# yli421/koopman-mpc-portfolio-rebalancing

Hardware: AMD Instinct MI355X
Metric: MPC window-solves/sec (batched backtest) at 1/2/4/8 MI355X vs host-CPU ref (higher is better)
Workload: dtype f32 rollout (fp32 GEMMs as three exact bf16 planes); mixed f32->f64 IPM solve (float32 phase to mu 3e-5, float64 finish: stopping rule, status and W in float64); 1 GPU; C3 (BASELINE configs[2]): 65536 windows/GPU, 100 assets, latent 256, H=10, obs 2000, GenericKM enc [1024,1024], L1-turnover MPC c=1e-3 tau=0.2 no-short; windows_per_gpu=65536, parallelism=1 GPU, no collective

## Files before the change

### koopman_mpc_portfolio_rebalancing_amd/csrc/kmpc_ipm_body.inc

```
    if constexpr (PH == 3) {
        if (reinterpret_cast<const int*>(args.warm + (size_t)b * args.warm_floats)[0] != 3) return;
    }
    const int nw = GL < 64 ? 1 : (MAXT <= 128 ? NWM : (int)(blockDim.x / WAVE));
    Reducer<HM, NWM, GL, Real> R(sh, nw);
    Thread<HM, MAXT, FL, CS, QL, GL, Real> T;
    T.bind_cold();
    T.H = EXACT ? HM : args.H;
    T.N = args.N;
    T.i = gvt<GL>();
    T.act = T.i < args.N;
    T.set_case(!args.allow_short, (args.c > Real(0.0)) || (args.tau > Real(0.0)), args.tau > Real(0.0));
    T.tau = args.tau;
    const int H = T.H, N = T.N;
    const double* wp = args.wp + (size_t)b * N;
    const float* yh = args.yhat + (size_t)yb * H * N;
    T.wpi = T.act ? wp[T.i] : Real(0.0);

    Real mx = Real(0.0);
    bool finite = true;
    bool r_zero = false;
    {
        Real rs[HM];
#pragma unroll
        for (int t = 0; t < HM; ++t) {
            T.m[t] = rs[t] = Real(0.0);
            if (T.act && t < H) {
                const float r = np_expf(yh[t * N + T.i]);
                T.m[t] = (Real)((double)r - 1.0);
                rs[t] = (Real)r;
                finite = finite && isfinite(T.m[t]);
            }
        }
        if (T.act) finite = finite && isfinite(T.wpi);
        R.periods(rs);
#pragma unroll
        for (int t = 0; t < HM; ++t) {
            r_zero = r_zero || (t < H && rs[t] == Real(0.0));
            if (T.act && t < H && rs[t] > Real(0.0) && rs[t] < Real(TINY_PERIOD))
                T.m[t] = (Real)((double)np_expf(yh[t * N + T.i]) / (double)rs[t] - 1.0);
            if (T.act && t < H) mx = fmax(mx, fabs(T.m[t]));
        }
        if (gvt<GL>() == 0) {
#pragma unroll
            for (int t = 0; t < HM; ++t)
                sh.lsc[t] = (t < H && rs[t] > Real(0.0) && rs[t] < Real(TINY_PERIOD)) ? (Real)log((double)rs[t]) : Real(0.0);
        }
    }
    mx = R.max1(mx);
    const Real nonfinite = R.max1(finite ? Real(0.0) : Real(1.0));
    Real sig = fmax(mx, Real(args.c));
    if (!(sig > Real(0.0))) sig = Real(1.0);
    T.sig = sig;
    T.isig = Real(1.0) / sig;
    T.irsig = Real(1.0) / sqrt(sig);
    T.c = Real(args.c) / sig;

    int status = KMPC_STATUS_SOLVER_ERROR;
    int it = 0;
    double* wout = args.wout + (size_t)b * (args.return_full ? H * N : N);
    const int tw = args.return_full ? H : 1;
    double best_obj = __builtin_nan("");
    bool handoff = false;
    int it0 = 0;

    if (nonfinite == Real(0.0) && isfinite(args.c) && isfinite(args.tau)) {
        if (r_zero) {
            status = KMPC_STATUS_INFEASIBLE;
        } else if (args.allow_short && !T.hs) {
            Real msum[HM];
#pragma unroll
            for (int t = 0; t < HM; ++t) msum[t] = (T.act && t < H) ? T.m[t] : Real(0.0);
            R.periods(msum);
            Real spread = Real(0.0);
#pragma unroll
            for (int t = 0; t < HM; ++t)
                if (T.act && t < H) spread = fmax(spread, fabs(T.m[t] - msum[t] / N));
            spread = R.max1(spread);
            if (spread == Real(0.0)) {
                const Real swp = R.sum1(T.act ? T.wpi : Real(0.0));
#pragma unroll
                for (int t = 0; t < HM; ++t) T.w[t] = swp != Real(0.0) ? T.wpi / swp : Real(1.0) / N;
                if constexpr (PH != 1) best_obj = record_best<HM, NWM>(T, R, wout, yh, args.c, tw);
                status = KMPC_STATUS_OPTIMAL;
            } else {
// ... 274 lines not shown
                }
                KMPC_PH(ph, 6);
            }
            __syncthreads();
            if (PH != 1 && best < huge_of<Real>()) {
                Real f = Real(0.0);
                for (int t = 0; t < H; ++t) f += log(sh.best_rw[t]) + sh.lsc[t] - args.c * sh.best_l1[t];
                best_obj = f;
            }
            if (best <= Real(1e-7)) status = KMPC_STATUS_OPTIMAL;
            else if (best <= Real(1e-4)) status = KMPC_STATUS_OPTIMAL_INACCURATE;
            else if (min_pr > Real(1e-6)) status = KMPC_STATUS_INFEASIBLE;
            else status = KMPC_STATUS_SOLVER_ERROR;
        }
    }
    if constexpr (PH == 1) {
        float* rec = args.warm + (size_t)b * args.warm_floats;
#ifdef KMPC_REG_HANDOFF
        hand_flag = handoff;
        if (handoff) {
#if KMPC_REG_HANDOFF_ON == 2
            float* hl = reinterpret_cast<float*>(kmpc_cold);
            const int ln = hand_lane<CS>();
#pragma unroll
            for (int t = 0; t < HM; ++t) {
                hl[(0 * HM + t) * CS + ln] = T.w[t];
                hl[(1 * HM + t) * CS + ln] = T.s[t];
                hl[(2 * HM + t) * CS + ln] = T.l1[t];
                hl[(3 * HM + t) * CS + ln] = T.l2[t];
                hl[(4 * HM + t) * CS + ln] = T.l3[t];
            }
            if (gvt<GL>() < HM) {
                hl[5 * HM * CS + gvt<GL>()] = sh.z4[gvt<GL>()];
                hl[5 * HM * CS + HM + gvt<GL>()] = sh.l4[gvt<GL>()];
                hl[5 * HM * CS + 2 * HM + gvt<GL>()] = sh.nu[gvt<GL>()];
            }
#else
#pragma unroll
            for (int t = 0; t < HM; ++t) {
                hand_w[t] = T.w[t];
                hand_s[t] = T.s[t];
                hand_l1[t] = T.l1[t];
                hand_l2[t] = T.l2[t];
                hand_l3[t] = T.l3[t];
            }
            if (gvt<GL>() < HM) {
                hand_z4 = sh.z4[gvt<GL>()];
                hand_l4 = sh.l4[gvt<GL>()];
                hand_nu = sh.nu[gvt<GL>()];
            }
#endif
        }
        if (false) {
#else
        if (handoff) {
#endif
            float* st = rec + WARM_HEAD;
#pragma unroll
            for (int t = 0; t < HM; ++t) {
                if (T.act && t < H) {
                    const int k = t * N + T.i;
                    st[k] = T.w[t];
                    st[H * N + k] = T.s[t];
                    st[2 * H * N + k] = T.l1[t];
                    st[3 * H * N + k] = T.l2[t];
                    st[4 * H * N + k] = T.l3[t];
                }
            }
            if (gvt<GL>() < H) {
                const int t = gvt<GL>();
                st[5 * H * N + t] = sh.z4[t];
                st[5 * H * N + H + t] = sh.l4[t];
                st[5 * H * N + 2 * H + t] = sh.nu[t];
            }
        }
        if (gvt<GL>() == 0) {
            int* hd = reinterpret_cast<int*>(rec);
            hd[0] = handoff ? 1 : 0;
            hd[1] = it;
        }
        return;
    }
    __syncthreads();
    const bool ok = status == KMPC_STATUS_OPTIMAL || status == KMPC_STATUS_OPTIMAL_INACCURATE;
    if (!ok && T.act) {
#pragma unroll
        for (int t = 0; t < HM; ++t)
            if (t < tw) wout[t * N + T.i] = T.wpi;
    }
    if (gvt<GL>() == 0) {
        args.obj[b] = ok ? best_obj : __builtin_nan("");
        args.status[b] = status;
        if constexpr (PH >= 2) {
            int* hd = reinterpret_cast<int*>(args.warm + (size_t)b * args.warm_floats);
            it0 = hd[1];
            if (PH == 2 && hd[0] == 1 && status != KMPC_STATUS_OPTIMAL) {
                hd[0] = 3;
                hd[1] = it + it0;
            }
        }
        if (args.iters) args.iters[b] = it + it0;
    }
```

### koopman_mpc_portfolio_rebalancing_amd/csrc/kmpc_solve_c3.hip

```cpp
#include "kmpc_solve_kernel.h"
#include "kmpc_bt_run.h"

#ifndef KMPC_REG_HANDOFF_ON
#define KMPC_REG_HANDOFF_ON 1
#endif

namespace kmpc {
template <int CS>
__device__ __forceinline__ int hand_lane() { const int t = (int)threadIdx.x; return t < CS ? t : CS - 1; }
}

namespace kmpc {
namespace {
template <int HM, int MAXT, bool EXACT, int FL, int CS, bool QL, int GL>
__global__ void __launch_bounds__(MAXT) __attribute__((amdgpu_waves_per_eu(1))) ipm_mixed_kernel(SolveArgs args) {
    constexpr int NWM = MAXT / WAVE;
    __shared__ union U {
        Shared<HM, NWM, float> f;
        Shared<HM, NWM, double> d;
    } shu;
    const int b = blockIdx.x;
    if (b >= args.B) return;
    const int yb = b;
#if KMPC_REG_HANDOFF_ON
    static_assert(KMPC_REG_HANDOFF_ON != 2 || (5 * HM * CS + 3 * HM) * 4 <= cold_bytes<HM, MAXT, CS, QL, GL, FL, double>(),
                  "the handoff fits the float64 cold arrays' LDS");
#if KMPC_REG_HANDOFF_ON == 1
    float hand_w[HM], hand_s[HM], hand_l1[HM], hand_l2[HM], hand_l3[HM];
    float hand_z4 = 1.0f, hand_l4 = 0.0f, hand_nu = 0.0f;
#endif
    bool hand_flag = false;
#define KMPC_REG_HANDOFF
#endif
    [&]() __attribute__((always_inline)) {
        constexpr int PH = 1;
        using Real = float;
        auto& sh = shu.f;
#include "kmpc_ipm_body.inc"
    }();
    __syncthreads();
    [&]() __attribute__((always_inline)) {
        constexpr int PH = 2;
        using Real = double;
        auto& sh = shu.d;
#include "kmpc_ipm_body.inc"
    }();
#undef KMPC_REG_HANDOFF
}
}

#ifndef KMPC_MIXED_FUSED
#define KMPC_MIXED_FUSED 1
#endif

size_t mixed_warm_floats(int H, int N) {
    return KMPC_MIXED_FUSED && KMPC_REG_HANDOFF_ON ? (size_t)WARM_HEAD : warm_stride(H, N);
}

int launch_ipm_c3(const SolveArgs& a, hipStream_t stream) {
    if (a.warm && KMPC_MIXED_FUSED) {
        const size_t lds = cold_bytes<10, 128, QL_CS, true, 64, 7, double>();
        hipLaunchKernelGGL((ipm_mixed_kernel<10, 128, true, 7, QL_CS, true, 64>), dim3(a.B), dim3(128), lds, stream, a);
        int rc = hipGetLastError() == hipSuccess ? KMPC_OK : KMPC_ERR_LAUNCH;
        if (rc == KMPC_OK) rc = launch_one<10, 128, true, 7, QL_CS, true, 64, 3>(a, 128, stream);
        return rc;
    }
    if (a.warm) {
        int rc = launch_one<10, 128, true, 7, QL_CS, true, 64, 1>(a, 128, stream);
        if (rc == KMPC_OK) rc = launch_one<10, 128, true, 7, QL_CS, true, 64, 2>(a, 128, stream);
        if (rc == KMPC_OK) rc = launch_one<10, 128, true, 7, QL_CS, true, 64, 3>(a, 128, stream);
        return rc;
    }
    return launch_one<10, 128, true, 7, QL_CS, true>(a, 128, stream);
}

int launch_bt_run_c3(const SolveArgs& a, int n_steps, int n_real, const float* yhat, const float* realized,
                     int step0, int S, double c, double* weights, double* value, double* hist, hipStream_t stream) {
    return launch_bt_run_one<10, 128, true, 7, QL_CS, true>(a, n_steps, n_real, yhat, realized, step0, S, c, weights,
                                                           value, hist, stream);
}
}

#ifdef KMPC_STATS
extern "C" int kmpc_debug_stats_c3(unsigned long long* out, int reset) { return kmpc::debug_stats_tu(out, reset); }
#endif
```

### koopman_mpc_portfolio_rebalancing_amd/csrc/kmpc_solve_c3sw.hip

```cpp
#include "kmpc_solve_kernel.h"
#include "kmpc_bt_sweep.h"

namespace kmpc {
int launch_bt_sweep_c3(const SolveArgs& a, const SweepLaunch& l, hipStream_t stream) {
    return launch_bt_sweep_one<10, 128, true, 7, QL_CS, true>(a, l, stream);
}
}
```

### koopman_mpc_portfolio_rebalancing_amd/csrc/kmpc_solve_kernel.h

```cpp
#pragma once
#include <hip/hip_runtime.h>
#include <math.h>
#include <stdint.h>

#include <type_traits>
#include <utility>

#include "kmpc_internal.h"
#include "kmpc_npexp.h"
#include "kmpc_solve_args.h"

namespace kmpc {

constexpr int WAVE = 64;
#ifdef KMPC_STATS
__device__ unsigned long long g_stats[2];
__device__ unsigned long long g_phase[16];
#ifndef KMPC_STATS_REAL
#define KMPC_STATS_REAL 0
#endif
struct PhaseClock {
    unsigned long long last;
    bool on;
    __device__ __forceinline__ void start(int real_bytes) {
// ... 235 lines not shown
}
__device__ __forceinline__ float bcast(float v, int src) { return as_f(__builtin_amdgcn_readlane(as_i(v), src)); }

template <int GL>
__device__ __forceinline__ int gvt() { return GL == 64 ? (int)threadIdx.x : (int)(threadIdx.x & (GL - 1)); }
template <int GL>
__device__ __forceinline__ int grp() { return GL == 64 ? 0 : (int)(threadIdx.x / GL); }
template <int GL>
__device__ __forceinline__ int glane() { return (int)(threadIdx.x & ((GL == 64 ? WAVE : GL) - 1)); }
template <int GL>
__device__ __forceinline__ int gwave() { return GL == 64 ? (int)(threadIdx.x / WAVE) : 0; }

template <int GL, class T>
__device__ __forceinline__ T group_sum(T v) {
    if constexpr (GL > 32) v = pair_sum<32>(v);
    if constexpr (GL > 16) v = pair_sum<16>(v);
    v = pair_sum<8>(v); v = pair_sum<4>(v); v = pair_sum<2>(v); v = pair_sum<1>(v);
    return v;
}
template <int GL, class T>
__device__ __forceinline__ T group_max(T v) {
    if constexpr (GL > 32) v = fmax(v, partner<32>(v));
    if constexpr (GL > 16) v = fmax(v, partner<16>(v));
    v = fmax(v, partner<8>(v)); v = fmax(v, partner<4>(v)); v = fmax(v, partner<2>(v)); v = fmax(v, partner<1>(v));
    return v;
}
template <int GL, class T>
__device__ __forceinline__ T group_min(T v) {
    if constexpr (GL > 32) v = fmin(v, partner<32>(v));
    if constexpr (GL > 16) v = fmin(v, partner<16>(v));
    v = fmin(v, partner<8>(v)); v = fmin(v, partner<4>(v)); v = fmin(v, partner<2>(v)); v = fmin(v, partner<1>(v));
    return v;
}
template <int C>
__device__ __forceinline__ double dpp_f64(double v) {
    const int2 x = as_i2(v);
    return as_f64(__builtin_amdgcn_mov_dpp(x.x, C, 0xf, 0xf, false),
                  __builtin_amdgcn_mov_dpp(x.y, C, 0xf, 0xf, false));
}
__device__ __forceinline__ double row_bcast(double v, int j) {
    switch (j & 15) {
        case 0: return dpp_f64<0x150>(v);
        case 1: return dpp_f64<0x151>(v);
        case 2: return dpp_f64<0x152>(v);
        case 3: return dpp_f64<0x153>(v);
        case 4: return dpp_f64<0x154>(v);
        case 5: return dpp_f64<0x155>(v);
        case 6: return dpp_f64<0x156>(v);
        case 7: return dpp_f64<0x157>(v);
        case 8: return dpp_f64<0x158>(v);
        case 9: return dpp_f64<0x159>(v);
        case 10: return dpp_f64<0x15a>(v);
        case 11: return dpp_f64<0x15b>(v);
        case 12: return dpp_f64<0x15c>(v);
        case 13: return dpp_f64<0x15d>(v);
        case 14: return dpp_f64<0x15e>(v);
        default: return dpp_f64<0x15f>(v);
    }
}
template <int C>
__device__ __forceinline__ float dpp_f32(float v) {
    return as_f(__builtin_amdgcn_mov_dpp(as_i(v), C, 0xf, 0xf, false));
}
__device__ __forceinline__ float row_bcast(float v, int j) {
    switch (j & 15) {
        case 0: return dpp_f32<0x150>(v);
        case 1: return dpp_f32<0x151>(v);
        case 2: return dpp_f32<0x152>(v);
        case 3: return dpp_f32<0x153>(v);
        case 4: return dpp_f32<0x154>(v);
        case 5: return dpp_f32<0x155>(v);
        case 6: return dpp_f32<0x156>(v);
        case 7: return dpp_f32<0x157>(v);
        case 8: return dpp_f32<0x158>(v);
        case 9: return dpp_f32<0x159>(v);
        case 10: return dpp_f32<0x15a>(v);
        case 11: return dpp_f32<0x15b>(v);
        case 12: return dpp_f32<0x15c>(v);
        case 13: return dpp_f32<0x15d>(v);
        case 14: return dpp_f32<0x15e>(v);
        default: return dpp_f32<0x15f>(v);
    }
}
template <int GL, class T>
__device__ __forceinline__ T gbcast(T v, int src) {
    if constexpr (GL == 64) {
        return bcast(v, src);
    } else if constexpr (GL == 16) {
        return row_bcast(v, src);
    } else {
        static_assert(GL == 32, "lane group of 16, 32 or 64");
        T a = row_bcast(v, src), b = a;
        swap16(a, b);
        return (src & 16) ? b : a;
    }
}

#ifndef KMPC_OPAQUE_LANE
#define KMPC_OPAQUE_LANE 1
#endif
#ifndef KMPC_RS_BANK
#define KMPC_RS_BANK 1
#endif
template <int M, int D, class T>
__device__ __forceinline__ void rs_level(T (&v)[M], int& n, int& slot) {
    if (n > 1) {
        const int h = n >> 1;
        const bool up = (threadIdx.x & D) != 0;
#pragma unroll
        for (int j = 0; j < (M > 1 ? M / 2 : 1); ++j) {
            if (j < h) {
                if constexpr (D == 32 || D == 16) {
                    T a = v[j], b = v[j + h];
                    if constexpr (D == 32) swap32(a, b); else swap16(a, b);
                    v[j] = a + b;
                } else if constexpr (KMPC_RS_BANK && (D == 8 || D == 4) && sizeof(T) == 4) {
                    constexpr int ctrl = D == 8 ? 0x140 : 0x141;
                    constexpr int lowm = D == 8 ? 0x3 : 0x5, upm = D == 8 ? 0xc : 0xa;
                    const int lo = as_i(v[j]), hi = as_i(v[j + h]);
                    const T t = as_f(__builtin_amdgcn_update_dpp(hi, lo, ctrl, 0xf, lowm, false));
                    const T u = as_f(__builtin_amdgcn_update_dpp(lo, hi, ctrl, 0xf, upm, false));
                    v[j] = t + u;
                } else if constexpr (KMPC_RS_BANK && (D == 8 || D == 4)) {
                    constexpr int ctrl = D == 8 ? 0x140 : 0x141;
                    constexpr int lowm = D == 8 ? 0x3 : 0x5, upm = D == 8 ? 0xc : 0xa;
                    const int2 lo = as_i2(v[j]), hi = as_i2(v[j + h]);
                    const double t = as_f64(__builtin_amdgcn_update_dpp(hi.x, lo.x, ctrl, 0xf, lowm, false),
                                            __builtin_amdgcn_update_dpp(hi.y, lo.y, ctrl, 0xf, lowm, false));
                    const double u = as_f64(__builtin_amdgcn_update_dpp(lo.x, hi.x, ctrl, 0xf, upm, false),
                                            __builtin_amdgcn_update_dpp(lo.y, hi.y, ctrl, 0xf, upm, false));
                    v[j] = t + u;
                } else {
                    const T lo = v[j], hi = v[j + h];
                    const T send = up ? lo : hi;
                    const T keep = up ? hi : lo;
                    v[j] = keep + dpp_partner<D>(send);
                }
            }
        }
        slot += up ? h : 0;
        n = h;
    } else {
        v[0] = pair_sum<D>(v[0]);
    }
}

template <int M, int GL = 64, class T>
__device__ __forceinline__ int wave_reduce_scatter(T (&v)[M]) {
    static_assert(M <= GL, "one slot per lane at most");
    int slot = 0, n = M;
    if constexpr (GL > 32) rs_level<M, 32>(v, n, slot);
    if constexpr (GL > 16) rs_level<M, 16>(v, n, slot);
    rs_level<M, 8>(v, n, slot);
    rs_level<M, 4>(v, n, slot);
    rs_level<M, 2>(v, n, slot);
    rs_level<M, 1>(v, n, slot);
    return slot;
}

template <class Real, int HM, int CS, bool LDS, int GL = 64>
struct Cold;
template <class Real, int HM, int CS, int GL>
struct Cold<Real, HM, CS, false, GL> {
    Real v[HM];
    __device__ __forceinline__ void bind(int) {}
    __device__ __forceinline__ Real operator[](int t) const { return v[t]; }
    __device__ __forceinline__ void set(int t, Real x) { v[t] = x; }
};
extern __shared__ double kmpc_cold[];
template <class Real, int HM, int CS, int GL>
struct Cold<Real, HM, CS, true, GL> {
    static constexpr int GS = GL < 64 ? CS / (64 / GL) : CS;
    int k;
    __device__ __forceinline__ void bind(int kk) { k = kk; }
    __device__ __forceinline__ static int lane() {
        const int tid = (int)threadIdx.x;
        if constexpr (GL < 64) {
            const int g = tid / GL, i = tid % GL;
            return g * GS + (i < GS ? i : GS - 1);
        } else {
            return tid < CS ? tid : CS - 1;
        }
// ... 640 lines not shown
            } else {
                r0[t] = r1[t] = Real(0.0);
            }
            rn = fmax(rn, fmax(fabs(r0[t]), fabs(r1[t])));
            if (gvt<TH::GLN>() == 0 && t < H) rn = fmax(rn, fabs(sh.b6[t] - sdw[t]));
            nl2 = (t < H) ? dl2 : Real(0.0);
            nl3 = (t < H) ? dl3 : Real(0.0);
        }
        if (!T.act) rn = Real(0.0);
        rn = R.max1(rn);
        KMPC_PH(np, 14);
        if (rn <= Real(REFINE_RTOL) * bn) break;
        if (gvt<TH::GLN>() < HM) {
            const int t = gvt<TH::GLN>();
            sh.lb5[t] = Real(0.0);
            sh.lb6[t] = (t < H) ? sh.b6[t] - sdw[t] : Real(0.0);
        }
        __syncthreads();
    }
#ifdef KMPC_STATS
    if (threadIdx.x == 0 && (KMPC_STATS_REAL == 0 || sizeof(Real) == KMPC_STATS_REAL)) {
        atomicAdd(&g_stats[0], (unsigned long long)r);
        atomicAdd(&g_stats[1], 1ull);
    }
#endif
    if (gvt<TH::GLN>() < HM) {
        const int t = gvt<TH::GLN>();
        const Real st = T.hs ? pxa * sh.isp1[t] : Real(0.0);
        const bool on = T.ht && t < H;
        sh.dz4[t] = on ? -st + sh.rg4[t] : Real(0.0);
        sh.dl4[t] = on ? (sh.b5[t] + sh.l4[t] * st) * sh.iz4[t] : Real(0.0);
    }
    KMPC_PH(np, 15);
}

template <int HM, int NWM, class TH, class Real = typename TH::real_t>
__device__ __forceinline__ Real max_step(const TH& T, Shared<HM, NWM, typename TH::real_t>& sh, Reducer<HM, NWM, TH::GLN, typename TH::real_t>& R,
                                           Real& c1, Real& c2) {
    const int H = T.H;
    Real a = huge_of<Real>(), mdw[HM];
    c1 = c2 = Real(0.0);
    Real DL1[HM], DL2[HM], DL3[HM];
    T.dual_dirs_all(DL1, DL2, DL3);
    Real qx = Real(0.0);
#pragma unroll
    for (int t = 0; t < HM; ++t) {
        mdw[t] = Real(0.0);
        if (t < H) {
            const Real dl1 = DL1[t], dl2 = DL2[t], dl3 = DL3[t];
            const Real d = T.w[t] - T.wprev(t);
            const Real dd = T.dw[t] - (t ? T.dw[t - 1] : Real(0.0));
            if (T.hw) {
                qx = fmax(qx, -T.dw[t] * T.iw[t]);
                a = to_bound(T.l1[t], dl1, a);
                c1 += T.w[t] * dl1 + T.l1[t] * T.dw[t];
                c2 += T.dw[t] * dl1;
            }
            if (T.hs) {
                const Real x2 = T.s[t] - d, dx2 = T.ds[t] - dd, x3 = T.s[t] + d, dx3 = T.ds[t] + dd;
                qx = fmax(qx, fmax(-dx2 * T.iz2[t], -dx3 * T.iz3[t]));
                a = to_bound(T.l2[t], dl2, a);
                a = to_bound(T.l3[t], dl3, a);
                c1 += x2 * dl2 + T.l2[t] * dx2 + x3 * dl3 + T.l3[t] * dx3;
                c2 += dx2 * dl2 + dx3 * dl3;
            }
            mdw[t] = T.m[t] * T.dw[t];
        }
    }
    if (qx > Real(0.0)) a = fmin(a, rcp_nr(qx));
    if (T.ht && (int)gvt<TH::GLN>() < H) {
        const int t = gvt<TH::GLN>();
        a = to_bound(sh.z4[t], sh.dz4[t], a);
        a = to_bound(sh.l4[t], sh.dl4[t], a);
        c1 += sh.z4[t] * sh.dl4[t] + sh.l4[t] * sh.dz4[t];
        c2 += sh.dz4[t] * sh.dl4[t];
    }
    a = R.periods_min_sums(mdw, a, c1, c2);
    Real qr = Real(0.0);
#pragma unroll
    for (int t = 0; t < HM; ++t)
        if (t < H) qr = fmax(qr, -mdw[t] * sh.iden[t]);
    if (qr > Real(0.0)) a = fmin(a, rcp_nr(qr));
    return a;
}

template <int HM, int NWM, class TH, class Real = typename TH::real_t>
__device__ __forceinline__ bool factor(TH& T, Shared<HM, NWM, typename TH::real_t>& sh, Reducer<HM, NWM, TH::GLN, typename TH::real_t>& R,
                                      PhaseClock& ph) {
    constexpr int KM = 3 * HM;
    constexpr int MC = Shared<HM, NWM>::MC;
    constexpr int RW = Shared<HM, NWM>::RW;
    const int H = T.H;
    Real E[HM], W1[HM], sp[HM];
#pragma unroll
    for (int t = 0; t < HM; ++t) {
        W1[t] = E[t] = T.P[t] = sp[t] = Real(0.0);
        Real iw = Real(0.0), iz2 = Real(0.0), iz3 = Real(0.0);
        if (T.act && t < H) {
            const Real d = T.w[t] - T.wprev(t);
            if (T.hw) { iw = rcp_nr(T.w[t]); W1[t] = T.l1[t] * iw; }
            if (T.hs) {
                iz2 = rcp_nr(T.s[t] - d);
                iz3 = rcp_nr(T.s[t] + d);
                const Real al = T.l2[t] * iz2, be = T.l3[t] * iz3;
                const Real P = rcp_nr(al + be);
                T.P[t] = P;
                E[t] = Real(4.0) * al * be * P;
                sp[t] = P;
            }
        }
        T.iw.set(t, iw);
        T.iz2.set(t, iz2);
        T.iz3.set(t, iz3);
    }
    const Real st_own = R.own1(sp);
    if (gvt<TH::GLN>() < HM) {
        const int t = gvt<TH::GLN>();
        const Real st = st_own;
        const Real ga = (T.ht && t < H) ? sh.l4[t] / sh.z4[t] : Real(0.0);
        const Real i1 = Real(1.0) / (Real(1.0) + ga * st);
        sh.rho[t] = (T.ht && t < H) ? ga * i1 : Real(0.0);
        sh.sr[t] = sqrt(sh.rho[t]);
        sh.sp[t] = t < H ? st : Real(0.0);
        sh.isp1[t] = i1;
        if (t == 0) sh.flag = 0;
    }
    bool ok = true;
    Real iDd[HM], Lr[HM];
    {
        Real pi = W1[0] + E[0];
#pragma unroll
        for (int t = 0; t < HM; ++t) {
            iDd[t] = Real(1.0);
            Lr[t] = Real(0.0);
            if (T.act && t < H) {
                if (t > 0) {
                    Lr[t] = E[t] * iDd[t - 1];
                    pi = W1[t] + Lr[t] * pi;
                }
                const Real dd = pi + ((t + 1 < HM && t + 1 < H) ? E[t + 1] : Real(0.0));
                ok = ok && (dd > Real(0.0)) && (dd < huge_of<Real>());
                iDd[t] = rcp_nr(dd);
            }
        }
#pragma unroll
        for (int t = 0; t < HM; ++t) {
            T.iDd.set(t, iDd[t]);
            T.Lr.set(t, Lr[t]);
        }
    }
    Real dq[HM];
#pragma unroll
    for (int k = HM - 1; k >= 0; --k) {
        Real v = Real(0.0);
        if (T.act && k < H) {
            v = iDd[k];
            if (k + 1 < HM) v += Lr[k + 1] * Lr[k + 1] * dq[k + 1];
        }
        dq[k] = v;
    }
    __syncthreads();
    if (!ok) sh.flag = 1;
    auto al = [&](int t) -> Real { return t < H ? T.m[t] * sh.iden[t] * T.irsig : Real(0.0); };
    auto ep = [&](int t) -> Real { return (t < H && T.ht) ? sh.sr[t] * T.bma(t) * T.P[t] : Real(0.0); };
    const int lane = glane<TH::GLN>(), wv = gwave<TH::GLN>();
    KMPC_PH(ph, 1);
// ... 63 lines not shown
        }
        __syncthreads();
#pragma unroll
        for (int k = 0; k < SPT; ++k) {
            const int s = gvt<TH::GLN>() + k * (TH::GLN == 64 ? (int)blockDim.x : TH::GLN);
            if (s < NS) {
                const int jl = kGramTab<HM>.v[s];
                const int j = jl & 255, l = jl >> 8;
                sh.G[j * KM + l] = tot[k];
                sh.G[l * KM + j] = tot[k];
            }
        }
    } else {
        Real qp[HM];
    #pragma unroll
        for (int r = 0; r < HM; ++r) qp[r] = Real(0.0);
        KMPC_PH(ph, 1);
        for (int c = 0; c < H; ++c) {
            Real qc[HM];
            Real dqc = Real(0.0), ac = Real(0.0), ec = Real(0.0);
    #pragma unroll
            for (int k = 0; k < HM; ++k) if (k == c) { dqc = dq[k]; ac = al(k); ec = ep(k); }
            {
                Real nxt = Real(0.0);
    #pragma unroll
                for (int r = HM - 1; r >= 0; --r) {
                    const Real v = (r == c) ? dqc : ((r < c && r + 1 < HM) ? Lr[r + 1] * nxt : Real(0.0));
                    qc[r] = v;
                    nxt = v;
                }
            }
            Real qcm1 = Real(0.0);
    #pragma unroll
            for (int k = 0; k + 1 < HM; ++k) if (k + 1 == c) qcm1 = qc[k];
            Real* rb = &sh.red[R.buf][0][0];
    #pragma unroll
            for (int k = 0; k < 3; ++k) {
                const Real cl = (k == 0) ? ac : ((k == 1) ? ec : Real(1.0));
                Real v[MC];
    #pragma unroll
                for (int q = 0; q < MC; ++q) {
                    Real x = Real(0.0);
                    if (q < KM) {
                        const int ty = q / HM, tj = q % HM;
                        if (tj <= c) {
                            Real base = qc[tj];
                            if (ty == 1 && tj >= 1) base -= qc[tj - 1];
                            if (k == 1) {
                                Real cross = (tj < c) ? qp[tj] : qcm1;
                                if (ty == 1 && tj >= 1) cross -= qp[tj - 1];
                                if (c == 0) cross = Real(0.0);
                                base -= cross;
                            }
                            const Real cj = (ty == 0) ? al(tj) : ((ty == 1) ? ep(tj) : Real(1.0));
                            x = cj * (cl * base);
                        }
                    }
                    v[q] = x;
                }
                const int slot = wave_reduce_scatter<MC, TH::GLN>(v);
                if ((lane & ((TH::GLN / MC) - 1)) == 0) rb[wv * RW + k * MC + slot] = v[0];
            }
            __syncthreads();
            for (int q = gvt<TH::GLN>(); q < 3 * MC; q += (TH::GLN == 64 ? (int)blockDim.x : TH::GLN)) {
                const int tyl = q / MC, j = q % MC;
                if (j < KM) {
                    const int tyj = j / HM, tj = j % HM;
                    if (tj < c || (tj == c && tyj <= tyl)) {
                        Real s = Real(0.0);
                        for (int w = 0; w < R.nw; ++w) s += rb[w * RW + q];
                        const int l = tyl * HM + c;
                        sh.G[j * KM + l] = s;
                        sh.G[l * KM + j] = s;
                    }
                }
            }
            R.buf ^= Shared<HM, NWM>::NB - 1;
    #pragma unroll
            for (int r = 0; r < HM; ++r) qp[r] = qc[r];
        }
    }
    __syncthreads();
    KMPC_PH(ph, 2);
    Real* col = &sh.red[0][0][0];
    if (gvt<TH::GLN>() < WAVE) {
        int r = lane;
#if KMPC_OPAQUE_LANE
        asm volatile("" : "+v"(r));
#endif
        const bool rused = r < KM && (r % HM) < H && (r / HM != 1 || T.ht);
        Real g[KM];
#pragma unroll
        for (int k = 0; k < KM; ++k) {
            const bool kused = (k % HM) < H && (k / HM != 1 || T.ht);
            Real v = (r < KM && k <= r && rused && kused) ? sh.G[r * KM + k] : Real(0.0);
            if (k == r) v += (k / HM < 2 || !rused) ? Real(1.0) : Real(0.0);
            g[k] = v;
        }
        bool bad = false;
        Real dinv = Real(0.0);
#pragma unroll
        for (int j = 0; j < KM; ++j) {
            const Real u = g[j];
            Real cv[KM];
            if (j + 1 < KM) {
                col[r] = u;
                __builtin_amdgcn_wave_barrier();
#pragma unroll
                for (int k = j + 1; k < KM; ++k) cv[k] = col[k];
            }
            const Real d = gbcast<TH::GLN>(u, j);
            bad = bad || !(d > Real(0.0)) || !(d < huge_of<Real>());
            const Real dm = fmax(d, tiny_of<Real>());
            Real id;
            if constexpr (sizeof(Real) == 8) {
                id = __builtin_amdgcn_rcp(dm);
                id = fma(id, fma(-dm, id, Real(1.0)), id);
                id = fma(id, fma(-dm, id, Real(1.0)), id);
            } else {
                id = __builtin_amdgcn_rcpf(dm);
            }
            const Real l = (r > j) ? u * id : Real(0.0);
            if (r == j) dinv = id;
            g[j] = l;
            if (j + 1 < KM) {
                __builtin_amdgcn_sched_barrier(0);
#pragma unroll
                for (int k = j + 1; k < KM; ++k) g[k] = fma(-l, cv[k], g[k]);
                __builtin_amdgcn_wave_barrier();
            }
        }
        if (r < KM) {
#pragma unroll
            for (int k = 0; k < KM; ++k) {
                const Real v = k < r ? g[k] : Real(0.0);
                sh.G[r * KM + k] = v;
            }
            sh.gid[r] = dinv;
        }
        if (bad && lane == 0) sh.flag = 1;
    }
    __syncthreads();
    KMPC_PH(ph, 3);
    return sh.flag == 0;
}

template <int HM, int NWM, class TH, class Real = typename TH::real_t>
__device__ __forceinline__ Real record_best(const TH& T, Reducer<HM, NWM, TH::GLN, typename TH::real_t>& R, double* wout,
                                              const float* yh, Real c, int tw) {
    const int H = T.H, N = T.N;
    Real rw[HM], l1n[HM];
#pragma unroll
    for (int t = 0; t < HM; ++t) {
        rw[t] = l1n[t] = Real(0.0);
        if (T.act && t < H) {
            if (t < tw) wout[t * N + T.i] = T.w[t];
            rw[t] = (Real(1.0) + T.m[t]) * T.w[t];
            l1n[t] = fabs(T.w[t] - T.wprev(t));
        }
    }
    R.periods(rw, l1n);
    Real f = Real(0.0);
#pragma unroll
    for (int t = 0; t < HM; ++t)
        if (t < H) f += log(rw[t]) + R.sh.lsc[t] - c * l1n[t];
    return f;
}

template <int HM, int MAXT, bool EXACT, int FL = -1, int CS = MAXT, bool QL = false, int GL = 64, int PH = 0>
__global__ void __launch_bounds__(MAXT)
__attribute__((amdgpu_waves_per_eu(PH == 1 ? KMPC_F32_WPE : (HM <= KMPC_WPE2_HM ? 2 : 1)))) ipm_kernel(SolveArgs args) {
    static_assert(3 * HM <= GL, "Schur system must fit one lane group");
    static_assert(GL == 64 || MAXT == 64, "lane groups pack one-wave blocks");
    using Real = std::conditional_t<PH == 1, float, double>;
    constexpr int NWM = MAXT / WAVE;
    constexpr int WPB = GL == 64 ? 1 : 64 / GL;
    static_assert(!cold_in_lds<HM, MAXT, CS, QL, GL, FL, Real>() ||
                  sizeof(Shared<HM, NWM, Real>) * WPB <= 9 * HM * HM * 8 + 16 * 1024, "cold_in_lds() LDS estimate");
    static_assert(sizeof(Shared<HM, NWM, Real>) * WPB + cold_bytes<HM, MAXT, CS, QL, GL, FL, Real>() <= 160 * 1024,
                  "LDS of one workgroup");
    __shared__ Shared<HM, NWM, Real> shv[WPB];
    auto& sh = shv[grp<GL>()];
    const int b = blockIdx.x * WPB + grp<GL>();
    if (b >= args.B) return;
    const int yb = b;
// ... 76 lines not shown
```

Baseline: 842,900 windows/s.

## Fuse float64 retry phase into mixed kernel and use DPP broadcasts in LDL

The float64 retry phase (PH 3) now runs inside the fused mixed-precision kernel, gated on an in-register retry flag, so the separate third kernel launch and its global warm-header read are no longer needed. Separately, the dense LDL factorization of the Schur complement replaces the per-column LDS write, wave barrier and reload with inline-asm v_fmac DPP row_newbcast updates that read column values straight from neighbouring lanes. The change adds code size and register pressure to the fused kernel, and relies on hand-written DPP asm with s_nop hazard padding for correctness.

```diff
diff --git a/koopman_mpc_portfolio_rebalancing_amd/csrc/kmpc_ipm_body.inc b/koopman_mpc_portfolio_rebalancing_amd/csrc/kmpc_ipm_body.inc
--- a/koopman_mpc_portfolio_rebalancing_amd/csrc/kmpc_ipm_body.inc
+++ b/koopman_mpc_portfolio_rebalancing_amd/csrc/kmpc_ipm_body.inc
@@ -1,5 +1,9 @@
     if constexpr (PH == 3) {
+#ifdef KMPC_FUSED_RETRY
+        if (!retry_flag) return;
+#else
         if (reinterpret_cast<const int*>(args.warm + (size_t)b * args.warm_floats)[0] != 3) return;
+#endif
     }
     const int nw = GL < 64 ? 1 : (MAXT <= 128 ? NWM : (int)(blockDim.x / WAVE));
     Reducer<HM, NWM, GL, Real> R(sh, nw);
@@ -440,6 +444,9 @@
         return;
     }
     __syncthreads();
+#ifdef KMPC_FUSED_RETRY
+    if constexpr (PH == 2) retry_flag = hand_flag && status != KMPC_STATUS_OPTIMAL;
+#endif
     const bool ok = status == KMPC_STATUS_OPTIMAL || status == KMPC_STATUS_OPTIMAL_INACCURATE;
     if (!ok && T.act) {
 #pragma unroll
diff --git a/koopman_mpc_portfolio_rebalancing_amd/csrc/kmpc_solve_c3.hip b/koopman_mpc_portfolio_rebalancing_amd/csrc/kmpc_solve_c3.hip
--- a/koopman_mpc_portfolio_rebalancing_amd/csrc/kmpc_solve_c3.hip
+++ b/koopman_mpc_portfolio_rebalancing_amd/csrc/kmpc_solve_c3.hip
@@ -1,8 +1,17 @@
+#ifndef KMPC_SCHUR_BCAST_F32
+#define KMPC_SCHUR_BCAST_F32 1
+#endif
+#ifndef KMPC_SCHUR_BCAST_F64
+#define KMPC_SCHUR_BCAST_F64 1
+#endif
 #include "kmpc_solve_kernel.h"
 #include "kmpc_bt_run.h"
 
 #ifndef KMPC_REG_HANDOFF_ON
 #define KMPC_REG_HANDOFF_ON 1
+#endif
+#ifndef KMPC_FUSED_RETRY_ON
+#define KMPC_FUSED_RETRY_ON (KMPC_REG_HANDOFF_ON != 0)
 #endif
 
 namespace kmpc {
@@ -39,12 +48,27 @@
 #include "kmpc_ipm_body.inc"
     }();
     __syncthreads();
+#if KMPC_FUSED_RETRY_ON
+    bool retry_flag = false;
+#define KMPC_FUSED_RETRY
+#endif
     [&]() __attribute__((always_inline)) {
         constexpr int PH = 2;
         using Real = double;
         auto& sh = shu.d;
 #include "kmpc_ipm_body.inc"
     }();
+#if KMPC_FUSED_RETRY_ON
+    if (!retry_flag) return;
+    __syncthreads();
+    [&]() __attribute__((always_inline)) {
+        constexpr int PH = 3;
+        using Real = double;
+        auto& sh = shu.d;
+#include "kmpc_ipm_body.inc"
+    }();
+#undef KMPC_FUSED_RETRY
+#endif
 #undef KMPC_REG_HANDOFF
 }
 }
@@ -62,7 +86,9 @@
         const size_t lds = cold_bytes<10, 128, QL_CS, true, 64, 7, double>();
         hipLaunchKernelGGL((ipm_mixed_kernel<10, 128, true, 7, QL_CS, true, 64>), dim3(a.B), dim3(128), lds, stream, a);
         int rc = hipGetLastError() == hipSuccess ? KMPC_OK : KMPC_ERR_LAUNCH;
+#if !KMPC_FUSED_RETRY_ON
         if (rc == KMPC_OK) rc = launch_one<10, 128, true, 7, QL_CS, true, 64, 3>(a, 128, stream);
+#endif
         return rc;
     }
     if (a.warm) {
diff --git a/koopman_mpc_portfolio_rebalancing_amd/csrc/kmpc_solve_c3sw.hip b/koopman_mpc_portfolio_rebalancing_amd/csrc/kmpc_solve_c3sw.hip
--- a/koopman_mpc_portfolio_rebalancing_amd/csrc/kmpc_solve_c3sw.hip
+++ b/koopman_mpc_portfolio_rebalancing_amd/csrc/kmpc_solve_c3sw.hip
@@ -1,3 +1,6 @@
+#ifndef KMPC_SCHUR_BCAST_F64
+#define KMPC_SCHUR_BCAST_F64 1
+#endif
 #include "kmpc_solve_kernel.h"
 #include "kmpc_bt_sweep.h"
 
diff --git a/koopman_mpc_portfolio_rebalancing_amd/csrc/kmpc_solve_kernel.h b/koopman_mpc_portfolio_rebalancing_amd/csrc/kmpc_solve_kernel.h
--- a/koopman_mpc_portfolio_rebalancing_amd/csrc/kmpc_solve_kernel.h
+++ b/koopman_mpc_portfolio_rebalancing_amd/csrc/kmpc_solve_kernel.h
@@ -341,6 +341,46 @@
         default: return dpp_f32<0x15f>(v);
     }
 }
+#define KMPC_FD(op, i) "\n\t" op " %[g" #i "], %[c" #i "], %[nl] row_newbcast:%[r" #i "] row_mask:0xf bank_mask:0xf"
+#define KMPC_FD_OUT(i) [g##i] "+v"(g[K0 + i])
+#define KMPC_FD_IN(i) [c##i] "v"(K0 + i < 16 ? ca : cb), [r##i] "n"((K0 + i) & 15)
+#define KMPC_FD_CHUNKS(op)                                                                                          \
+    if constexpr (CNT == 8)                                                                                         \
+        asm("s_nop 1" KMPC_FD(op, 0) KMPC_FD(op, 1) KMPC_FD(op, 2) KMPC_FD(op, 3) KMPC_FD(op, 4)                    \
+            KMPC_FD(op, 5) KMPC_FD(op, 6) KMPC_FD(op, 7)                                                            \
+            : KMPC_FD_OUT(0), KMPC_FD_OUT(1), KMPC_FD_OUT(2), KMPC_FD_OUT(3), KMPC_FD_OUT(4),                       \
+              KMPC_FD_OUT(5), KMPC_FD_OUT(6), KMPC_FD_OUT(7)                                                        \
+            : [nl] "v"(nl), KMPC_FD_IN(0), KMPC_FD_IN(1), KMPC_FD_IN(2), KMPC_FD_IN(3), KMPC_FD_IN(4),              \
+              KMPC_FD_IN(5), KMPC_FD_IN(6), KMPC_FD_IN(7));                                                         \
+    else if constexpr (CNT == 4)                                                                                    \
+        asm("s_nop 1" KMPC_FD(op, 0) KMPC_FD(op, 1) KMPC_FD(op, 2) KMPC_FD(op, 3)                                   \
+            : KMPC_FD_OUT(0), KMPC_FD_OUT(1), KMPC_FD_OUT(2), KMPC_FD_OUT(3)                                        \
+            : [nl] "v"(nl), KMPC_FD_IN(0), KMPC_FD_IN(1), KMPC_FD_IN(2), KMPC_FD_IN(3));                            \
+    else if constexpr (CNT == 2)                                                                                    \
+        asm("s_nop 1" KMPC_FD(op, 0) KMPC_FD(op, 1)                                                                 \
+            : KMPC_FD_OUT(0), KMPC_FD_OUT(1) : [nl] "v"(nl), KMPC_FD_IN(0), KMPC_FD_IN(1));                         \
+    else                                                                                                            \
+        asm("s_nop 1" KMPC_FD(op, 0) : KMPC_FD_OUT(0) : [nl] "v"(nl), KMPC_FD_IN(0))
+template <int CNT, int K0, int KM>
+__device__ __forceinline__ void fmac_dpp_chunk(float (&g)[KM], float ca, float cb, float nl) {
+    KMPC_FD_CHUNKS("v_fmac_f32_dpp");
+}
+template <int CNT, int K0, int KM>
+__device__ __forceinline__ void fmac_dpp_chunk(double (&g)[KM], double ca, double cb, double nl) {
+    KMPC_FD_CHUNKS("v_fmac_f64_dpp");
+}
+#undef KMPC_FD_CHUNKS
+#undef KMPC_FD_IN
+#undef KMPC_FD_OUT
+#undef KMPC_FD
+template <int K0, int KM, class T>
+__device__ __forceinline__ void fmac_dpp_from(T (&g)[KM], T ca, T cb, T nl) {
+    constexpr int n = KM - K0, CNT = n >= 8 ? 8 : (n >= 4 ? 4 : (n >= 2 ? 2 : 1));
+    if constexpr (n > 0) {
+        fmac_dpp_chunk<CNT, K0>(g, ca, cb, nl);
+        fmac_dpp_from<K0 + CNT>(g, ca, cb, nl);
+    }
+}
 template <int GL, class T>
 __device__ __forceinline__ T gbcast(T v, int src) {
     if constexpr (GL == 64) {
@@ -357,6 +397,12 @@
 
 #ifndef KMPC_OPAQUE_LANE
 #define KMPC_OPAQUE_LANE 1
+#endif
+#ifndef KMPC_SCHUR_BCAST_F32
+#define KMPC_SCHUR_BCAST_F32 0
+#endif
+#ifndef KMPC_SCHUR_BCAST_F64
+#define KMPC_SCHUR_BCAST_F64 0
 #endif
 #ifndef KMPC_RS_BANK
 #define KMPC_RS_BANK 1
@@ -1163,6 +1209,33 @@
         if (t < H) qr = fmax(qr, -mdw[t] * sh.iden[t]);
     if (qr > Real(0.0)) a = fmin(a, rcp_nr(qr));
     return a;
+}
+
+template <int J, int KM, class Real>
+__device__ __forceinline__ void ldl_steps_dpp(Real (&g)[KM], int r, bool& bad, Real& dinv) {
+    static_assert(KM <= 32, "the column sits on two DPP rows");
+    if constexpr (J < KM) {
+        Real u = g[J];
+        if constexpr (J > 0) asm("s_nop 1" : "+v"(u));
+        Real ca = u, cb = u;
+        if constexpr (KM > 16 && J + 1 < KM) swap16(ca, cb);
+        const Real d = bcast(u, J);
+        bad = bad || !(d > Real(0.0)) || !(d < huge_of<Real>());
+        const Real dm = fmax(d, tiny_of<Real>());
+        Real id;
+        if constexpr (sizeof(Real) == 8) {
+            id = __builtin_amdgcn_rcp(dm);
+            id = fma(id, fma(-dm, id, Real(1.0)), id);
+            id = fma(id, fma(-dm, id, Real(1.0)), id);
+        } else {
+            id = __builtin_amdgcn_rcpf(dm);
+        }
+        const Real l = (r > J) ? u * id : Real(0.0);
+        if (r == J) dinv = id;
+        g[J] = l;
+        fmac_dpp_from<J + 1>(g, ca, cb, -l);
+        ldl_steps_dpp<J + 1>(g, r, bad, dinv);
+    }
 }
 
 template <int HM, int NWM, class TH, class Real = typename TH::real_t>
@@ -1392,6 +1465,8 @@
     }
     __syncthreads();
     KMPC_PH(ph, 2);
+    constexpr bool DPPCOL = TH::GLN == 64 && KM <= 32 &&
+                            (sizeof(Real) == 4 ? KMPC_SCHUR_BCAST_F32 != 0 : KMPC_SCHUR_BCAST_F64 != 0);
     Real* col = &sh.red[0][0][0];
     if (gvt<TH::GLN>() < WAVE) {
         int r = lane;
@@ -1409,8 +1484,9 @@
         }
         bool bad = false;
         Real dinv = Real(0.0);
-#pragma unroll
-        for (int j = 0; j < KM; ++j) {
+        if constexpr (DPPCOL) ldl_steps_dpp<0>(g, r, bad, dinv);
+#pragma unroll
+        for (int j = DPPCOL ? KM : 0; j < KM; ++j) {
             const Real u = g[j];
             Real cv[KM];
             if (j + 1 < KM) {
```

New measurement: 872,400 windows/s, median of 6. 3.5% higher.
